# WGLab/NanoRepeat

Hardware: NVIDIA B200
Metric: GCUPS (higher is better)
Workload: dtype u16x2 (2*score + mark + 64 per half, two reads per word); s32 (score*65536 - span) for reads > 384 bases

## Files before the change

include/nanorepeat_b200.h:

```cpp
#ifndef NANOREPEAT_B200_H
#define NANOREPEAT_B200_H

#include <stdint.h>

#ifdef __cplusplus
extern "C" {
#endif

#define NR_OK                0
#define NR_ERR_CUDA         -1
#define NR_ERR_ARG          -2
#define NR_ERR_BAD_BASE     -3
#define NR_ERR_TOO_LARGE    -4
#define NR_ERR_NOMEM        -5
#define NR_ERR_UNKNOWN_TYPE -6

typedef struct nr_scoring_t {
    int32_t match;
    int32_t mismatch;
    int32_t gap_open1;
    int32_t gap_ext1;
    int32_t gap_open2;
    int32_t gap_ext2;
    int32_t ambiguous;
// ... 10 lines not shown
} nr_rung_t;

typedef struct nr_stats_t {
    int64_t algorithmic_cells;
    int64_t executed_cells;
    int64_t n_tasks;
    int32_t kernel_launches;
    int32_t n_skipped;
    int64_t h2d_bytes;
    int64_t d2h_bytes;
} nr_stats_t;

typedef struct nr_launch_info_t {
    int64_t paired_cells;
    int64_t rest_cells;
    int32_t n_pairs;
    int32_t n_rest;
    int32_t n_redo;
    int32_t reserved;
    float paired_ms, rest_ms, redo_ms;
    float reserved2;
    int64_t paired_useful_cells;
    int64_t rest_useful_cells;
} nr_launch_info_t;

int nr_get_preset(const char* data_type, nr_scoring_t* out);

int nr_init(int device);
int nr_shutdown(void);
const char* nr_last_error(void);
int nr_device_info(int32_t* device, int32_t* sm_count, int32_t* clock_khz);

int nr_limits(int32_t* max_score, int32_t* max_tlen);

int nr_set_ladder_mode(int mode);

int nr_score_tasks(const nr_scoring_t* sc, int32_t n_tasks,
                   const char* const* queries, const int32_t* qlen,
                   const char* const* targets, const int32_t* tlen,
                   nr_aln_t* out);

int nr_round2_region(const nr_scoring_t* sc,
                     const char* left, int32_t n_left, const char* motif, int32_t motif_len, int32_t T,
                     int32_t n_reads, const char* const* cores, const int32_t* core_len,
                     nr_aln_t* out);

// ... 97 lines not shown
```

nanorepeat_b200/csrc/nr_api.cu:

```cuda
#include "../../include/nanorepeat_b200.h"
#include "nr_launch.h"

#include <algorithm>
#if defined(__x86_64__)
#include <tmmintrin.h>
#endif
#include <atomic>
#include <chrono>
#include <cstdarg>
#include <cstdio>
#include <cstdlib>
#include <cstring>
#include <functional>
#include <mutex>
#include <new>
#include <string>
#include <thread>
#include <memory>
#include <unordered_map>
#include <vector>

namespace {

thread_local std::string g_err;
thread_local int g_code = 0;
thread_local nr_stats_t g_last_stats = {};
// ... 242 lines not shown
    std::vector<nr::Task> tasks;
    std::vector<nr::LadderTask> ltasks;
    std::vector<nr::LadderRegion> lregs;
    bool ladder = false;
    bool flag = false;
    bool pair = false;
    bool r2flags = false;
    std::vector<nr::pr::Pair2> pairs2;
    std::vector<nr::pr::Pair3> pairs3;
    int n_pairs2_single = 0, n_pairs3_single = 0;
    bool long_redone = false;
    int n_long_pairs = 0;
    void* d_pairs = nullptr;
    uint2* d_prung = nullptr;
    size_t prung_bytes = 0;
    int32_t* d_redo = nullptr;
    size_t redo_bytes = 0;
    cudaEvent_t ev_t[6] = {};
    bool timed[3] = {};
    int* h_redo_count = nullptr;
    int* h_spin = nullptr;
    long long paired_cells = 0, rest_cells = 0;
    long long paired_useful = 0, rest_useful = 0;
    size_t n_out = 0;
    std::vector<int32_t> order;
    std::vector<nr::CoopInfo> coop;
    std::vector<int32_t> coop_idx;
    nr::CoopInfo* d_coop = nullptr;
    int32_t* d_coop_idx = nullptr;
    std::vector<int32_t> lt_src;
    uint32_t* d_state = nullptr;
    size_t state_bytes = 0;
    int* d_flags = nullptr;
    size_t flags_bytes = 0;
    Launch launch = {};
    Pool pool;
    std::vector<RegionInfo> regions;
    int n_reads = 0;
    int n_skipped = 0;
    int n_ambiguous_reads = 0;
    std::vector<int32_t> read_region;
    std::vector<int32_t> kmin, kmax;
    std::vector<int64_t> rung_off;
    void* d_blob = nullptr;
    size_t blob_bytes = 0;
    void* h_blob = nullptr;
    nr::Task* d_tasks = nullptr;
    nr::LadderTask* d_ltasks = nullptr;
    nr::LadderRegion* d_lregs = nullptr;
    int32_t* d_order = nullptr;
    uint32_t* d_pool = nullptr;
    int* d_counters = nullptr;
    int4* d_out = nullptr;
    size_t out_bytes = 0;
// ... 52 lines not shown
    return k;
}

size_t align_up(size_t x, size_t a) { return (x + a - 1) / a * a; }

struct PhaseTrace {
    const bool on = getenv("NR_TRACE") != nullptr;
    std::chrono::steady_clock::time_point t0 = std::chrono::steady_clock::now();
    void mark(const char* what) {
        if (!on) return;
        const auto t1 = std::chrono::steady_clock::now();
        fprintf(stderr, "[nr trace] %-28s %8.1f us   (ends at %10.1f us, thread %04x)\n", what,
                std::chrono::duration<double, std::micro>(t1 - t0).count(), std::fmod(std::chrono::duration<double, std::micro>(t1.time_since_epoch()).count(), 1e8),
                (unsigned)(std::hash<std::thread::id>()(std::this_thread::get_id()) & 0xffff));
        t0 = t1;
    }
};

bool is_map_ont(const nr_scoring_t& c) {
    return c.match == 2 && c.mismatch == 4 && c.gap_open1 == 4 && c.gap_ext1 == 2 && c.gap_open2 == 24 && c.gap_ext2 == 1 &&
           c.ambiguous == 1;
}

template <class Key, class Emit>
void make_pairs(std::vector<int>& ids, Key key, Emit emit) {
    std::vector<uint64_t> w(ids.size());
    for (size_t i = 0; i < ids.size(); ++i) w[i] = ((uint64_t)(uint32_t)key(ids[i]) << 32) | (uint32_t)~(uint32_t)ids[i];
    std::sort(w.begin(), w.end(), std::greater<uint64_t>());
    for (size_t i = 0; i < w.size(); ++i) ids[i] = (int)~(uint32_t)w[i];
    for (size_t i = 0; i < ids.size(); i += 2) emit(ids[i], i + 1 < ids.size() ? ids[i + 1] : -1);
}

int plan_batch(nr_batch* b) {
    const bool ladder = b->ladder;
    const int n = ladder ? (int)b->ltasks.size() : (int)b->tasks.size();
    if (b->kind != KIND_ROUND3) b->n_out = b->tasks.size();
    b->stats = {};
    b->stats.n_tasks = (int64_t)b->n_out;
    std::vector<long long> cost(n, 0);
    std::vector<int> task_R(n, nr::kMinR), task_ns(n, 1), task_sweep(n, 0), task_rungs(n, 0);
    std::vector<char> paired(n, 0);
    const int max_r = ladder ? nr::kMaxRLadder : nr::kMaxRExact;
    const bool fixed = is_map_ont(b->sc);
    PhaseTrace trace;
    for (int i = 0; i < n; ++i) {
        int q_len, t_len, t_sweep;
// ... 11 lines not shown
        } else {
            const nr::Task& t = b->tasks[i];
            q_len = t.q_len;
            t_len = t_sweep = t.t_len;
            if (t_len > 0) b->stats.algorithmic_cells += (long long)q_len * t_len;
        }
        if (q_len <= 0 || t_len <= 0) {
            paired[i] = 2;
            if (t_len < 0) ++b->n_skipped;
            continue;
        }
        long long m = (long long)b->sc.match * std::min(q_len, t_len);
        if (m > kMaxScore || t_len > kMaxTlen) {
            paired[i] = 2;
            ++b->n_skipped;
            continue;
        }
        nr::stripe_shape(q_len, max_r, task_R[i], task_ns[i]);
        task_sweep[i] = t_sweep;
        cost[i] = (long long)task_ns[i] * 32 * task_R[i] * t_len;
    }
    trace.mark("task shapes");
    std::vector<long long> pair_cost;
    Launch& L = b->launch;
    L = {};
    long long state_off = 0;
    long long rung_off = 0;
    if (b->pair && fixed && !ladder && b->kind == KIND_ROUND2) {
        for (const RegionInfo& g : b->regions) {
            std::vector<int> ids;
            for (int r = g.first_read; r < g.first_read + g.n_reads; ++r) {
                const nr::Task& t = b->tasks[r];
                if (!paired[r] && t.q_len >= 1 && t.q_len <= 32 * nr::pr::kMaxRPair2 && t.t_len >= 1) ids.push_back(r);
            }
            make_pairs(ids, [&](int i) { return b->tasks[i].q_len; }, [&](int x, int y) {
                const int R = nr::pr::pair_rows(b->tasks[x].q_len);
                nr::pr::Pair2 p = {x, y, g.n_left, -1};
                if (g.n_left >= 2 && state_off + nr::pr::state_words(R) < 0x7fffffffLL) {
                    p.state_off = (int32_t)state_off;
                    state_off += nr::pr::state_words(R);
                }
                b->pairs2.push_back(p);
                paired[x] = 1;
                if (y >= 0) paired[y] = 1;
                L.pair_R = std::max(L.pair_R, R);
                pair_cost.push_back((long long)32 * R * b->tasks[x].t_len);
                b->paired_useful += (long long)(b->tasks[x].q_len + (y >= 0 ? b->tasks[y].q_len : 0)) * b->tasks[x].t_len;
            });
        }
    } else if (b->pair && fixed && ladder && b->flag) {
        if (b->qsrc && !b->qsrc->pairs2.empty() && (int)b->lt_src.size() == n) {
            const nr_batch* src = b->qsrc;
            std::vector<int> src2lt(src->tasks.size(), -1);
            for (int i = 0; i < n; ++i)
                if (b->lt_src[i] >= 0) src2lt[b->lt_src[i]] = i;
            for (int pi = 0; pi < src->n_pairs2_single; ++pi) {
                const nr::pr::Pair2& p2 = src->pairs2[pi];
                int la = src2lt[p2.a], lb = p2.b >= 0 ? src2lt[p2.b] : -1;
                if (la >= 0 && paired[la]) la = -1;
                if (lb >= 0 && paired[lb]) lb = -1;
                if (la < 0 && lb < 0) continue;
                const nr::LadderRegion& g = b->lregs[b->ltasks[la >= 0 ? la : lb].region];
                if (g.n_left <= 0 || g.n_right <= 0) continue;
                const int q = std::max(src->tasks[p2.a].q_len, p2.b >= 0 ? src->tasks[p2.b].q_len : 0);
                const int R = nr::pr::pair_rows(q);
                int kmin = INT32_MAX, kmax = -1;
                for (int t : {la, lb})
                    if (t >= 0) { kmin = std::min(kmin, b->ltasks[t].kmin); kmax = std::max(kmax, b->ltasks[t].kmax); }
                nr::pr::Pair3 p = {la, lb, (int32_t)rung_off, -1, R, {0, 0, 0}};
                if (p2.state_off >= 0 && src->d_state && g.n_left >= 2 && g.n_left == p2.mark_col) p.state_off = p2.state_off;
// ... 21 lines not shown
                if (y >= 0) { kmin = std::min(kmin, b->ltasks[y].kmin); kmax = std::max(kmax, b->ltasks[y].kmax); }
                nr::pr::Pair3 p = {x, y, (int32_t)rung_off, -1, 0, {0, 0, 0}};
                rung_off += kmax - kmin + 1;
                b->pairs3.push_back(p);
                paired[x] = 1;
                if (y >= 0) paired[y] = 1;
                const int R = nr::pr::pair_rows(tx.q_len);
                L.pair_R = std::max(L.pair_R, R);
                pair_cost.push_back((long long)32 * R * (g.n_right + g.n_left + (long long)g.m * kmax));
                b->paired_useful += (long long)(tx.q_len + (y >= 0 ? b->ltasks[y].q_len : 0)) * (g.n_right + g.n_left + (long long)g.m * kmax);
            });
            i0 = i1;
        }
        if (rung_off > 0x7fffffffLL) return fail(NR_ERR_TOO_LARGE, "more than 2^31 rungs in one batch");
        L.redo_R = L.pair_R;
    }
    trace.mark("pairing");
    b->state_bytes = sizeof(uint32_t) * 32 * (size_t)state_off;
    L.n_pairs = (int)pair_cost.size();
    if (L.n_pairs) {
        std::vector<int> po(L.n_pairs);
        {
            std::vector<uint64_t> w(L.n_pairs);
            for (int i = 0; i < L.n_pairs; ++i) w[i] = ((uint64_t)pair_cost[i] << 24) | (uint32_t)(0xffffff - i);
            std::sort(w.begin(), w.end(), std::greater<uint64_t>());
            for (int i = 0; i < L.n_pairs; ++i) po[i] = 0xffffff - (int)(w[i] & 0xffffff);
        }
        if (!b->pairs2.empty()) { std::vector<nr::pr::Pair2> t(L.n_pairs); for (int i = 0; i < L.n_pairs; ++i) t[i] = b->pairs2[po[i]]; b->pairs2.swap(t); }
        else { std::vector<nr::pr::Pair3> t(L.n_pairs); for (int i = 0; i < L.n_pairs; ++i) t[i] = b->pairs3[po[i]]; b->pairs3.swap(t); }
        for (long long c : pair_cost) b->paired_cells += 2 * c;
        b->stats.executed_cells += b->paired_cells;
        L.pair_blocks = std::max(1, std::min(g_ctx.sm_count, L.n_pairs));
    }
    trace.mark("pair order");
    b->n_pairs2_single = (int)b->pairs2.size();
    struct LongPair { int a, b, n_left; long long cost; };
    std::vector<LongPair> long_pairs;
    long long long_pair_rows = 0;
    b->n_pairs3_single = (int)b->pairs3.size();
    if (b->pair && fixed && ladder && b->flag && !getenv("NR_NO_LONG_PAIRS")) {
        for (int i0 = 0; i0 < n;) {
            int i1 = i0;
            while (i1 < n && b->ltasks[i1].region == b->ltasks[i0].region) ++i1;
            const nr::LadderRegion& g = b->lregs[b->ltasks[i0].region];
            std::vector<int> ids;
            if (g.n_left > 0 && g.n_right > 0)
                for (int i = i0; i < i1; ++i)
// ... 216 lines not shown
    const size_t order_bytes = sizeof(int32_t) * n_rest;
    const size_t pair_bytes = b->pairs2.empty() ? sizeof(nr::pr::Pair3) * b->pairs3.size() : sizeof(nr::pr::Pair2) * b->pairs2.size();
    const size_t pool_bytes = sizeof(uint32_t) * (b->pool.words.size() + 4);
    const size_t coop_bytes = sizeof(nr::CoopInfo) * b->coop.size();
    const size_t cidx_bytes = b->coop.empty() ? 0 : sizeof(int32_t) * b->coop_idx.size();
    const size_t off_reg = align_up(task_bytes, 256);
    const size_t off_order = off_reg + align_up(reg_bytes, 256);
    const size_t off_pair = off_order + align_up(order_bytes, 256);
    const size_t off_coop = off_pair + align_up(pair_bytes, 256);
    const size_t off_cidx = off_coop + align_up(coop_bytes, 256);
    const size_t off_pool = off_cidx + align_up(cidx_bytes, 256);
    const size_t off_cnt = off_pool + align_up(pool_bytes, 256);
    b->blob_bytes = off_cnt + 256;
    b->out_bytes = sizeof(int4) * std::max<size_t>(b->n_out, 1);
    b->scratch_bytes = sizeof(int4) * scratch_total;
    int rc;
    if ((rc = cached_alloc(&b->d_blob, b->blob_bytes, BUF_DEV))) return rc;
    if ((rc = cached_alloc(&b->h_blob, b->blob_bytes, BUF_PIN))) return rc;
    if ((rc = cached_alloc((void**)&b->d_out, b->out_bytes, BUF_DEV))) return rc;
    if ((rc = cached_alloc((void**)&b->h_out, b->out_bytes, BUF_PIN))) return rc;
    if (scratch_total && (rc = cached_alloc((void**)&b->d_scratch, b->scratch_bytes, BUF_SCRATCH))) return rc;
    if (b->flags_bytes && (rc = cached_alloc((void**)&b->d_flags, b->flags_bytes, BUF_DEV))) return rc;
    if (b->state_bytes && (rc = cached_alloc((void**)&b->d_state, b->state_bytes, BUF_DEV))) return rc;
    if (b->flag) {
        b->sel_bytes = sizeof(int4) * std::max<size_t>((size_t)b->n_reads, 1);
        if ((rc = cached_alloc((void**)&b->d_sel, b->sel_bytes, BUF_DEV))) return rc;
        if ((rc = cached_alloc((void**)&b->h_sel, b->sel_bytes, BUF_PIN))) return rc;
    }
    if (!b->pairs3.empty()) {
        b->redo_bytes = sizeof(int32_t) * (size_t)n * 2;
        if ((rc = cached_alloc((void**)&b->d_prung, b->prung_bytes, BUF_DEV))) return rc;
        if ((rc = cached_alloc((void**)&b->d_redo, b->redo_bytes, BUF_DEV))) return rc;
        if ((rc = cached_alloc((void**)&b->h_redo_count, 64, BUF_PIN))) return rc;
        b->h_redo_count[0] = b->h_redo_count[1] = 0;
    }
    trace.mark("buffers (cached alloc)");
    char* h = static_cast<char*>(b->h_blob);
    char* d = static_cast<char*>(b->d_blob);
    if (task_bytes) memcpy(h, ladder ? (const void*)b->ltasks.data() : (const void*)b->tasks.data(), task_bytes);
    if (reg_bytes) memcpy(h + off_reg, b->lregs.data(), reg_bytes);
    if (order_bytes) memcpy(h + off_order, b->order.data(), order_bytes);
    if (coop_bytes) memcpy(h + off_coop, b->coop.data(), coop_bytes);
    if (cidx_bytes) memcpy(h + off_cidx, b->coop_idx.data(), cidx_bytes);
    if (pair_bytes) memcpy(h + off_pair, b->pairs2.empty() ? (const void*)b->pairs3.data() : (const void*)b->pairs2.data(), pair_bytes);
    if (!b->pool.words.empty()) memcpy(h + off_pool, b->pool.words.data(), pool_bytes - 16);
    memset(h + off_pool + pool_bytes - 16, 0, 16);
// ... 97 lines not shown
        if (b->qsrc->run_stream != st) CUDA_TRY(cudaStreamWaitEvent(st, b->qsrc->ev_done, 0));
    }
    CUDA_TRY(cudaMemsetAsync(b->d_counters, 0, 32 * sizeof(int), st));
    if (b->flags_bytes) CUDA_TRY(cudaMemsetAsync(b->d_flags, 0, b->flags_bytes, st));
    int launches = 0;
    int rc;
    const bool timing = g_timing.load() != 0;
    if (timing)
        for (cudaEvent_t& e : b->ev_t)
            if (!e) CUDA_TRY(cudaEventCreate(&e));
    b->timed[0] = b->timed[1] = b->timed[2] = false;
    auto mark = [&](int i, cudaStream_t s) { return timing ? cudaEventRecord(b->ev_t[i], s) : cudaSuccess; };
    if (L.n_pairs || b->n_long_pairs) {
        const bool ladder_batch = L.ladder;
        nr::RestArgs ra;
        if ((rc = rest_args(b, b->d_order, L.count, st, &ra))) return rc;
        int wpb = kWarpsPerBlock;
        if (const char* e = getenv("NR_WPB")) wpb = std::max(4, std::min(kWarpsPerBlock, atoi(e)));
        const int blocks = std::max(1, std::min(g_ctx.sm_count, L.count + L.n_pairs));
        nr::pr::Deal deal = nr::pr::make_deal(L.count, L.n_pairs, wpb, blocks);
        if (getenv("NR_PLAIN_DEAL")) deal.nb_long = -1;
        CUDA_TRY(mark(2, st));
        if (!ladder_batch) {
            const int stride = exact_smem_int4(std::max(L.pair_R, L.R));
            const size_t smem = (size_t)wpb * stride * sizeof(int4);
            if (smem > nrl::kMaxDynShared) return fail(NR_ERR_ARG, "launch needs %zu bytes of shared memory", smem);
            CUDA_TRY(nrl::launch_pair_round2(blocks, wpb * 32, smem, st, static_cast<const nr::pr::Pair2*>(b->d_pairs), deal, b->d_tasks,
                                             ra, b->d_pool, k, b->d_counters, stride, b->d_out, b->d_state));
        } else {
            const int stride = pair_ladder_smem_int4(L.pair_R, L.R);
            const size_t smem = (size_t)wpb * stride * sizeof(int4);
            if (smem > nrl::kMaxDynShared) return fail(NR_ERR_ARG, "launch needs %zu bytes of shared memory", smem);
            CUDA_TRY(nrl::launch_pair_ladder(blocks, wpb * 32, smem, st, static_cast<const nr::pr::Pair3*>(b->d_pairs), deal, b->d_ltasks,
                                             ra, b->qsrc ? b->qsrc->d_pool : b->d_pool, b->d_pool, b->d_lregs, k, b->d_counters, stride,
                                             b->d_prung, b->d_out, b->d_sel, b->d_counters + 2, b->d_redo,
                                             b->qsrc ? b->qsrc->d_state : nullptr));
        }
        CUDA_TRY(cudaGetLastError());
        CUDA_TRY(mark(3, st));
        b->timed[1] = timing;
        ++launches;
        if (!b->pairs3.empty()) {
            CUDA_TRY(mark(4, st));
            if ((rc = launch_rest(b, st, k, b->d_redo, 0, std::max(1, std::min(g_ctx.sm_count, 2 * L.n_pairs)), L.redo_R,
                                  b->d_counters + 2, b->d_counters + 3))) return rc;
            CUDA_TRY(mark(5, st));
            b->timed[2] = timing;
            CUDA_TRY(cudaMemcpyAsync(b->h_redo_count, b->d_counters + 2, sizeof(int), cudaMemcpyDeviceToHost, st));
            CUDA_TRY(cudaMemcpyAsync(b->h_redo_count + 1, b->d_counters + 4, sizeof(int), cudaMemcpyDeviceToHost, st));
            ++launches;
        }
// ... 356 lines not shown
    g_ladder_mode.store(mode);
    return NR_OK;
}

int nr_limits(int32_t* max_score, int32_t* max_tlen) {
    if (max_score) *max_score = kMaxScore;
    if (max_tlen) *max_tlen = kMaxTlen;
    return NR_OK;
}

void nr_batch_destroy(nr_batch_t* b) {
    if (!b) return;
    if (--b->refs > 0) return;
    if (b->committed && b->ev_uploaded) cudaEventSynchronize(b->ev_uploaded);
    if (b->ran && b->ev_done) cudaEventSynchronize(b->ev_done);
    else if (b->ran && b->run_stream) cudaStreamSynchronize(b->run_stream);
    cached_free(b->d_blob, b->blob_bytes, BUF_DEV);
    cached_free(b->h_blob, b->blob_bytes, BUF_PIN);
    cached_free(b->d_out, b->out_bytes, BUF_DEV);
    cached_free(b->h_out, b->out_bytes, BUF_PIN);
    cached_free(b->d_scratch, b->scratch_bytes, BUF_SCRATCH);
    cached_free(b->d_flags, b->flags_bytes, BUF_DEV);
    cached_free(b->d_state, b->state_bytes, BUF_DEV);
    cached_free(b->d_sel, b->sel_bytes, BUF_DEV);
    cached_free(b->h_sel, b->sel_bytes, BUF_PIN);
    cached_free(b->d_prung, b->prung_bytes, BUF_DEV);
    cached_free(b->d_redo, b->redo_bytes, BUF_DEV);
    cached_free(b->h_redo_count, 64, BUF_PIN);
    cached_free(b->h_spin, 64, BUF_PIN);
    nr_batch* src = b->qsrc;
    free_events(b);
    delete b;
    if (src) nr_batch_destroy(src);
}

nr_batch_t* nr_batch_begin_round3_from(nr_batch_t* round2) {
    if (!round2 || round2->kind != KIND_ROUND2 || !round2->committed) {
        fail(NR_ERR_ARG, "nr_batch_begin_round3_from: needs a committed round-2 batch");
        return nullptr;
    }
    nr_batch* b = new_batch(&round2->sc, KIND_ROUND3);
    if (!b) return nullptr;
    if (!b->ladder) {
        fail(NR_ERR_ARG, "nr_batch_begin_round3_from: needs a ladder mode (nr_set_ladder_mode 1 or 2)");
        free_events(b);
        delete b;
// ... 223 lines not shown
                rg.score = a.x;
                rg.starts_in_left = in_left;
                rg.ends_in_right = in_right;
                rg.pad[0] = rg.pad[1] = 0;
            }
            if (top > 0 && a.x == top && in_left) { sum += k; ++cnt; }
        }
        sum_k[r] = sum;
        n_k[r] = cnt;
        top_score[r] = top;
    }
    return NR_OK;
}

int nr_set_timing(int on) {
    g_timing.store(on ? 1 : 0);
    return NR_OK;
}

int nr_batch_launch_info(nr_batch_t* b, nr_launch_info_t* out) {
    if (!b || !out) return fail(NR_ERR_ARG, "nr_batch_launch_info: NULL argument");
    if (!b->committed) return fail(NR_ERR_ARG, "nr_batch_launch_info: batch was not committed");
    *out = {};
    out->paired_cells = b->paired_cells;
    out->rest_cells = b->rest_cells;
    out->paired_useful_cells = b->paired_useful;
    out->rest_useful_cells = b->rest_useful;
    out->n_pairs = b->launch.n_pairs;
    out->n_rest = b->launch.count;
    if (b->ran) {
        CUDA_TRY(cudaEventSynchronize(b->ev_done));
        if (b->h_redo_count) out->n_redo = *b->h_redo_count;
        if (b->timed[0]) CUDA_TRY(cudaEventElapsedTime(&out->rest_ms, b->ev_t[0], b->ev_t[1]));
        if (b->timed[1]) CUDA_TRY(cudaEventElapsedTime(&out->paired_ms, b->ev_t[2], b->ev_t[3]));
        if (b->timed[2]) CUDA_TRY(cudaEventElapsedTime(&out->redo_ms, b->ev_t[4], b->ev_t[5]));
    }
    return NR_OK;
}

int nr_batch_stats(const nr_batch_t* b, nr_stats_t* out) {
    if (!b || !out) return fail(NR_ERR_ARG, "nr_batch_stats: NULL argument");
    *out = b->stats;
    return NR_OK;
}

int nr_last_stats(nr_stats_t* out) {
    if (!out) return fail(NR_ERR_ARG, "nr_last_stats: NULL argument");
    *out = g_last_stats;
    return NR_OK;
}

int nr_score_tasks(const nr_scoring_t* sc, int32_t n_tasks, const char* const* queries, const int32_t* qlen,
                   const char* const* targets, const int32_t* tlen, nr_aln_t* out) {
    if (n_tasks > 0 && !out) return fail(NR_ERR_ARG, "nr_score_tasks: out is NULL");
// ... 295 lines not shown
```

nanorepeat_b200/csrc/nr_launch.h:

```cpp
#pragma once
#include "nr_kernels.cuh"
#include "nr_pair_kernels.cuh"

namespace nrl {

constexpr size_t kMaxDynShared = (size_t)nr::kWarpsPerBlock * 14 * 1024;

cudaError_t launch_exact(bool fixed, int blocks, int threads, size_t smem, cudaStream_t st, const nr::Task* tasks,
                         const nr::RestArgs& ra, const uint32_t* pool, const nr::ScoreW& k, int* counter, int stride, int4* out);
cudaError_t launch_ladder(bool flag, int blocks, int threads, size_t smem, cudaStream_t st, const nr::LadderTask* tasks,
                          const nr::RestArgs& ra, const int* n_order_dev, const uint32_t* qpool, const uint32_t* pool,
                          const nr::LadderRegion* regs, const nr::ScoreW& k, int* counter, int stride, int4* out, int4* sel);
cudaError_t launch_pair_round2(int blocks, int threads, size_t smem, cudaStream_t st, const nr::pr::Pair2* pairs,
                               const nr::pr::Deal& deal, const nr::Task* tasks, const nr::RestArgs& ra, const uint32_t* pool,
                               const nr::ScoreW& k, int* counter, int stride, int4* out, uint32_t* state);
cudaError_t launch_pair_ladder(int blocks, int threads, size_t smem, cudaStream_t st, const nr::pr::Pair3* pairs,
                               const nr::pr::Deal& deal, const nr::LadderTask* tasks, const nr::RestArgs& ra,
                               const uint32_t* qpool, const uint32_t* pool, const nr::LadderRegion* regs, const nr::ScoreW& k,
                               int* counter, int stride, uint2* prung, int4* out, int4* sel, int* redo_count, int32_t* redo,
                               const uint32_t* qstate);

template <class F>
inline cudaError_t prepare(F fn, bool& done) {
    if (done) return cudaSuccess;
    cudaError_t e = cudaFuncSetAttribute(fn, cudaFuncAttributeMaxDynamicSharedMemorySize, (int)kMaxDynShared);
    if (e == cudaSuccess) e = cudaFuncSetAttribute(fn, cudaFuncAttributePreferredSharedMemoryCarveout, cudaSharedmemCarveoutMaxShared);
    if (e == cudaSuccess) done = true;
    return e;
}

}
```

nanorepeat_b200/csrc/nr_launch_pair2.cu:

```cuda
#define NR_DEFINE_PAIR_ROUND2_KERNEL
#include "nr_launch.h"
#include <mutex>
namespace nrl {
cudaError_t launch_pair_round2(int blocks, int threads, size_t smem, cudaStream_t st, const nr::pr::Pair2* pairs,
                               const nr::pr::Deal& deal, const nr::Task* tasks, const nr::RestArgs& ra, const uint32_t* pool,
                               const nr::ScoreW& k, int* counter, int stride, int4* out, uint32_t* state) {
    static std::mutex mu;
    static bool done = false;
    {
        std::lock_guard<std::mutex> lk(mu);
        cudaError_t e = prepare(nr::pr::pair_round2_kernel, done);
        if (e != cudaSuccess) return e;
    }
    nr::pr::pair_round2_kernel<<<blocks, threads, smem, st>>>(pairs, deal, tasks, ra, pool, k, counter, stride, out, state);
    return cudaGetLastError();
}
}
```

nanorepeat_b200/csrc/nr_pair_kernels.cuh:

```cuda
#pragma once
#include "nr_kernels.cuh"

namespace nr {
namespace pr {

typedef unsigned u32;
constexpr int kBias = 64;
__host__ __device__ constexpr u32 pk2(int hi, int lo) { return ((u32)(hi & 0xffff) << 16) | (u32)(lo & 0xffff); }
__host__ __device__ constexpr u32 pk(int v) { return pk2(v, v); }
__host__ __device__ constexpr u32 sub2(int v) { return 0u - (((u32)v << 16) | (u32)v); }

constexpr int kMatch = 4, kMismatch = 8, kAmbiguous = 2, kOpen1 = 12, kExt1 = 4, kOpen2 = 50, kExt2 = 2, kRefund1 = 8, kRefund2 = 48;
constexpr u32 kFloorFwd = pk(kBias + 1);
constexpr u32 kFloorBwd = pk(kBias);
constexpr u32 kOnes = 0x00010001u;

__device__ __forceinline__ u32 pmadd(u32 a, u32 mul, u32 b) {
    u32 d;
    asm("mad.lo.u32 %0, %1, %2, %3;" : "=r"(d) : "r"(a), "r"(mul), "r"(b));
    return d;
}

template <u32 FLOOR>
__device__ __forceinline__ void cell(u32 hd, u32 s, u32 one, u32& h, u32& e1, u32& e2, u32& f1, u32& f2) {
    const u32 d = __viaddmax_u16x2(hd, s, FLOOR);
    const u32 t = __vimax3_u16x2(d, e1, e2);
    h = __vimax3_u16x2(t, f1, f2);
    e1 = __viaddmax_u16x2(h, pk(-kOpen1), pmadd(e1, one, sub2(kExt1)));
    e2 = __viaddmax_u16x2(h, pk(-kOpen2), pmadd(e2, one, sub2(kExt2)));
    f1 = __viaddmax_u16x2(h, pk(-kOpen1), pmadd(f1, one, sub2(kExt1)));
    f2 = __viaddmax_u16x2(h, pk(-kOpen2), pmadd(f2, one, sub2(kExt2)));
}

struct Pair2 {
    int32_t a, b;
    int32_t mark_col;
    int32_t state_off;
};

struct Pair3 {
    int32_t a, b;
    int32_t rung_off;
    int32_t state_off;
    int32_t R;
    int32_t pad[3];
};

__host__ __device__ constexpr int state_words(int R) { return 3 * R + 1; }

template <int R>
__device__ __forceinline__ void build_profile(uint4* prof, const uint32_t* __restrict__ qa, int q_a,
                                              const uint32_t* __restrict__ qb, int q_b, int row0, int lane, bool reverse) {
    constexpr int CH = StripeCfg<R>::CH;
    u32* p = reinterpret_cast<u32*>(prof);
    const uint32_t amb_a = q_a > 0 ? read_ambiguity_plane(qa, q_a) : 0u, amb_b = q_b > 0 ? read_ambiguity_plane(qb, q_b) : 0u;
#pragma unroll
    for (int r = 0; r < 4 * CH; ++r) {
        const int i = row0 + r;
        int ca = 4, cb = 4;
        if (r < R && i < q_a) {
            const int qi = reverse ? q_a - 1 - i : i;
// ... 25 lines not shown
    int* spin;
    int4 bcur;
    ulonglong2 bnxt;
    const ulonglong2* tok_in;
    ulonglong2* tok_out;
    const u32* bstage;
    int b_stride, brow0;
    const int* bdone;
    int bdone_need;
    bool late_pending;
    u32* bsm_w;
    const uint4* prof;
    const uint32_t* twords;
    int t_len, lane;
    int mark_col;
    int q_a, q_b;
    const u32* bsm;
    uint2* rung_out;
    int jnext, m, kcnt, zone_start;
    int col0;
    const u32* resume;
    u32* save;
    int save_col;
    u32 H[R], E1[R], E2[R];
    u32 hup_prev, h_out, f1_out, f2_out;
    u32 best;
    u32 bestc, raw_hi, raw_lo;
    int st_hi, st_lo;
    u32 nz, bz;
    uint32_t twl, w0, w1;
    int wi, wmax, wsh;
    const char* prof_lane;
    u32 tokP, tokJ;

    __device__ __forceinline__ uint32_t tword(int i) const { return __ldg(&twords[min(max(i, 0), wmax)]); }

    __device__ __forceinline__ void init() {
        if (MODE == kPF && resume) {
#pragma unroll
            for (int r = 0; r < R; ++r) {
                H[r] = __ldcg(&resume[r * 32 + lane]);
                E1[r] = __ldcg(&resume[(R + r) * 32 + lane]);
                E2[r] = __ldcg(&resume[(2 * R + r) * 32 + lane]);
            }
            hup_prev = lane ? __ldcg(&resume[(R - 1) * 32 + lane - 1]) : FLOOR;
            best = __ldcg(&resume[3 * R * 32 + lane]);
// ... 224 lines not shown
            if (MULTI && bot && lane == 31) store_bnd(&bnd_out[jj], (int)h_out, (int)f1_out, (int)f2_out, tag_out);
        }
    }

    __device__ __forceinline__ void slow_until(int& st, int end, u32 one, unsigned four) {
#pragma unroll 1
        for (; st < end; ++st) {
            if (MULTI && MODE == kPF && late_pending && st >= zone_start) late_load();
            if ((st & 15) == 0) refill();
            step<false, true>(st, one, four);
        }
    }

#ifndef NR_PAIR3_UNROLL
#define NR_PAIR3_UNROLL 2
#endif
#ifndef NR_PAIR2_UNROLL
#define NR_PAIR2_UNROLL 4
#endif
#ifndef NR_PAIR2_MULTI_UNROLL
#define NR_PAIR2_MULTI_UNROLL 4
#endif
    static constexpr int kUnroll = MODE == kP2 ? (MULTI ? NR_PAIR2_MULTI_UNROLL : NR_PAIR2_UNROLL) : (MULTI ? 1 : NR_PAIR3_UNROLL);
    template <bool TRACK, bool SPECIAL = false>
    __device__ __forceinline__ void fast_until(int& st, int end, u32 one, unsigned four) {
        for (; st + 16 <= end; st += 16) {
            refill();
#pragma unroll 1
            for (int b = 0; b < 16; b += kUnroll) {
#pragma unroll
                for (int u = 0; u < kUnroll; ++u) step<true, TRACK, SPECIAL>(st + b + u, one, four);
            }
        }
    }

    __device__ __forceinline__ void run(u32 one, unsigned four, int zone_start_) {
        init();
        zone_start = zone_start_;
        const int n = t_len - col0;
        const int nsteps = n + 31;
        const int inside_end = ((n - 1) >> 4) << 4;
        const int mc = mark_col - col0;
        int st = 0;
        slow_until(st, min(32, nsteps), one, four);
        if (MODE == kPB) {
            fast_until<true>(st, inside_end, one, four);
        } else if (MODE == kP2) {
            if (mc >= 0) {
                const int zs = max(mc - 2, 0);
                const int before = st;
                fast_until<false>(st, min(inside_end, (zs >> 4) << 4), one, four);
                if (st != before) {
                    const u32 nb = __vmaxu2(bestc, best | kOnes);
                    const u32 x = nb ^ bestc;
                    bestc = nb;
                    if (x > 0xffffu) { st_hi = lane; raw_hi = 0; }
                    if (x & 0xffffu) { st_lo = lane; raw_lo = 0; }
                }
                slow_until(st, min(nsteps, ((mc + 32 + 15) >> 4) << 4), one, four);
            }
            fast_until<true>(st, inside_end, one, four);
        } else {
            const int first = min(zone_start, mc >= 0 ? mc : zone_start);
            fast_until<true>(st, min(inside_end, (first >> 4) << 4), one, four);
            if (MULTI && late_pending && st + 16 <= inside_end) late_load();
            fast_until<true, true>(st, inside_end, one, four);
        }
        slow_until(st, nsteps, one, four);
    }
};

constexpr int kMaxRPair3 = 16;
constexpr int kMaxRPair2 = kMaxRPair3;
constexpr int kPairEntry = 1 << 30;

__host__ __device__ __forceinline__ int pair_rows(int q_len) {
    int R = (q_len + 31) / 32;
    return R < kMinR ? kMinR : R;
}

struct Deal {
    int n_rest, n_pairs;
    int static_rest;
    int nb_long;
// ... 23 lines not shown
    }
    if (first) {
        first = false;
        const int wpb = blockDim.x >> 5, warp = threadIdx.x >> 5, blk = (int)blockIdx.x;
        if (blk < dl.nb_long) {
            const int e = blk * wpb + warp;
            if (e < dl.static_rest) return e;
        } else {
            const int p = warp * ((int)gridDim.x - dl.nb_long) + (blk - dl.nb_long);
            if (p < dl.static_pairs) return dl.n_rest + p;
        }
    }
    int d = 0;
    if ((threadIdx.x & 31) == 0) d = atomicAdd(counter, 1);
    d = __shfl_sync(kFull, d, 0);
    const int rest_left = dl.n_rest - dl.static_rest;
    if (d < rest_left) return dl.static_rest + d;
    const int p = dl.static_pairs + d - rest_left;
    return p < dl.n_pairs ? dl.n_rest + p : -1;
}

template <int R>
__device__ __forceinline__ void pair2_task(const Pair2& pt, const Task* __restrict__ tasks, const uint32_t* __restrict__ pool,
                                           uint4* prof, int lane, u32 one, unsigned four, int4* out, u32* state) {
    const Task ta = tasks[pt.a];
    Task tb = ta;
    int q_b = 0;
    if (pt.b >= 0) { tb = tasks[pt.b]; q_b = tb.q_len; }
    __syncwarp();
    build_profile<R>(prof, pool + ta.q_word, ta.q_len, pool + tb.q_word, q_b, lane * R, lane, false);
    __syncwarp();
    Sweep<R, kP2> sw;
    sw.prof = prof; sw.twords = pool + ta.t_word; sw.t_len = ta.t_len; sw.lane = lane;
    sw.mark_col = pt.mark_col;
    sw.col0 = 0; sw.resume = nullptr;
    sw.save_col = pt.mark_col - 2;
    sw.save = (state && pt.state_off >= 0 && sw.save_col >= 0) ? state + (size_t)pt.state_off * 32 : nullptr;
    sw.run(one, four, 0);
#pragma unroll
    for (int half = 0; half < 2; ++half) {
        const u32 cls = half ? (sw.bestc & 0xffffu) : (sw.bestc >> 16);
        const u32 raw = half ? (sw.raw_lo & 0xffffu) : (sw.raw_hi >> 16);
        const int st = half ? sw.st_lo : sw.st_hi;
        const int score = (int)(cls - (kBias + 1)) >> 1;
        const int col = st - lane;
        unsigned key = 0;
        if (score > 0) key = ((unsigned)score << 17) | ((0xffffu - (unsigned)col) << 1) | (raw & 1u);
        key = __reduce_max_sync(kFull, key);
        const int tid = half ? pt.b : pt.a;
        if (lane == 0 && tid >= 0) {
            int4 rec = make_int4(0, 0, 0, 0);
            if (key) {
                const int c = 0xffff - (int)((key >> 1) & 0xffffu);
                const bool inside = c <= pt.mark_col || !(key & 1u);
                rec = make_int4((int)(key >> 17), inside ? 0 : pt.mark_col + 1, c + 1, 0);
            }
            out[tid] = rec;
        }
    }
}

// ... 47 lines not shown
                if (key) {
                    const int c = 0xffff - (int)((key >> 1) & 0xffffu);
                    const bool inside = c <= pt.mark_col || !(key & 1u);
                    rec = make_int4((int)(key >> 17), inside ? 0 : pt.mark_col + 1, c + 1, 0);
                }
                out[tid] = rec;
            }
        }
    }
}

template <int R>
__device__ __forceinline__ void pair2_stripe_dispatch(int r, const Pair2& pt, int s, const Task* __restrict__ tasks,
                                                      const uint32_t* __restrict__ pool, const RestArgs& ra, uint4* prof, int lane,
                                                      u32 one, unsigned four, int4* out) {
    if constexpr (is_coop_height(R))
        if (r == R) { pair2_stripe<R>(pt, s, tasks, pool, ra, prof, lane, one, four, out); return; }
    if constexpr (R < kMaxRLadder) pair2_stripe_dispatch<R + 1>(r, pt, s, tasks, pool, ra, prof, lane, one, four, out);
}

template <int R>
__device__ __forceinline__ void pair2_dispatch(int r, const Pair2& pt, const Task* __restrict__ tasks,
                                               const uint32_t* __restrict__ pool, uint4* prof, int lane, u32 one,
                                               unsigned four, int4* out, u32* state) {
    if (r == R) { pair2_task<R>(pt, tasks, pool, prof, lane, one, four, out, state); return; }
    if constexpr (R < kMaxRPair2) pair2_dispatch<R + 1>(r, pt, tasks, pool, prof, lane, one, four, out, state);
}

#ifdef NR_DEFINE_PAIR_ROUND2_KERNEL
__global__ void __launch_bounds__(32 * kWarpsPerBlock, 1)
pair_round2_kernel(const Pair2* __restrict__ pairs, Deal dl, const Task* __restrict__ tasks, RestArgs ra,
                   const uint32_t* __restrict__ pool, ScoreW scw, int* counter, int smem_stride, int4* out, u32* state) {
    extern __shared__ uint4 psmem[];
    const ScoreView<true> sc(scw);
    const int lane = threadIdx.x & 31, warp = threadIdx.x >> 5;
    uint4* prof = psmem + warp * smem_stride;
    bool first = true;
    for (;;) {
        const int i = next_item(dl, first, counter);
        if (i < 0) break;
        if (i < ra.n_order) {
            const int e = ra.order[i];
            if (e & kPairEntry) {
                const Pair2 mp = pairs[(e & ~kPairEntry) >> kCodeBits];
                pair2_stripe_dispatch<kMinR>(ra.coop[mp.state_off].rows, mp, (e & ((1 << kCodeBits) - 1)) - 1, tasks, pool, ra, prof, lane,
                                             (u32)sc.one, sc.four, out);
            } else {
                exact_entry(e, tasks, pool, sc, ra, reinterpret_cast<int4*>(prof), lane, out);
            }
            continue;
        }
        const Pair2 pt = pairs[i - ra.n_order];
        int q = tasks[pt.a].q_len;
        if (pt.b >= 0) q = max(q, tasks[pt.b].q_len);
        pair2_dispatch<kMinR>(pair_rows(q), pt, tasks, pool, prof, lane, (u32)sc.one, sc.four, out, state);
    }
}
#endif

__device__ __forceinline__ void rung_of(u32 P, u32 J, u32 rc, int& score, bool& in_right, bool& unmarked) {
    const u32 np = max(J, rc);
    const int s_p = (int)(P - kBias) >> 1;
    const int s_np = (int)(np - 2 * kBias) >> 1;
    in_right = s_np > s_p;
    score = max(s_p, s_np);
    unmarked = np & 1u;
}

__device__ __forceinline__ void pair3_select(const Pair3& pt, const LadderTask& ta, const LadderTask& tb, int kmin, u32 rcand,
                                             const uint2* rungs, int lane, int min_score, int4* sel, int* redo_count, int32_t* redo,
                                             int redo_shift) {
#pragma unroll
    for (int half = 0; half < 2; ++half) {
        const int tid = half ? pt.b : pt.a;
        if (tid < 0) continue;
        const LadderTask& tk = half ? tb : ta;
        const u32 rc = half ? (rcand & 0xffffu) : (rcand >> 16);
        int top = 0;
// ... 227 lines not shown
```

nanorepeat_b200/engine.py:

```python
import ctypes
import itertools
import os

import numpy as np

_HERE = os.path.dirname(os.path.abspath(__file__))
LIB_PATH = os.path.join(_HERE, "libnanorepeat_b200.so")

NR_OK = 0
ERROR_NAMES = {-1: "NR_ERR_CUDA", -2: "NR_ERR_ARG", -3: "NR_ERR_BAD_BASE", -4: "NR_ERR_TOO_LARGE",
               -5: "NR_ERR_NOMEM", -6: "NR_ERR_UNKNOWN_TYPE"}


class Scoring(ctypes.Structure):
    _fields_ = [(n, ctypes.c_int32) for n in
                ("match", "mismatch", "gap_open1", "gap_ext1", "gap_open2", "gap_ext2", "ambiguous", "min_dp_score")]


class Stats(ctypes.Structure):
    _fields_ = [("algorithmic_cells", ctypes.c_int64), ("executed_cells", ctypes.c_int64),
                ("n_tasks", ctypes.c_int64), ("kernel_launches", ctypes.c_int32), ("n_skipped", ctypes.c_int32),
                ("h2d_bytes", ctypes.c_int64), ("d2h_bytes", ctypes.c_int64)]

    def as_dict(self):
        return {n: int(getattr(self, n)) for n, _ in self._fields_ if n != "reserved"}


class LaunchInfo(ctypes.Structure):
    _fields_ = [("paired_cells", ctypes.c_int64), ("rest_cells", ctypes.c_int64), ("n_pairs", ctypes.c_int32),
                ("n_rest", ctypes.c_int32), ("n_redo", ctypes.c_int32), ("reserved", ctypes.c_int32),
                ("paired_ms", ctypes.c_float), ("rest_ms", ctypes.c_float), ("redo_ms", ctypes.c_float),
                ("reserved2", ctypes.c_float), ("paired_useful_cells", ctypes.c_int64), ("rest_useful_cells", ctypes.c_int64)]

    def as_dict(self):
        return {n: getattr(self, n) for n, _ in self._fields_ if not n.startswith("reserved")}


class RegionIn(ctypes.Structure):
    _fields_ = [("left", ctypes.c_char_p), ("n_left", ctypes.c_int32), ("right", ctypes.c_char_p), ("n_right", ctypes.c_int32),
                ("motif", ctypes.c_char_p), ("motif_len", ctypes.c_int32), ("n_reads", ctypes.c_int32),
                ("reads", ctypes.c_void_p), ("reads_len", ctypes.c_int64),
                ("dist_between_anchors", ctypes.POINTER(ctypes.c_int32)),
                ("has_round1_max_dist", ctypes.c_int32), ("round1_max_dist", ctypes.c_int64)]


ALN_DTYPE = np.dtype([("score", "<i4"), ("tstart", "<i4"), ("tend", "<i4")])
RUNG_DTYPE = np.dtype([("score", "<i4"), ("starts_in_left", "u1"), ("ends_in_right", "u1"), ("pad", "u1", (2,))])


class GmmParams(ctypes.Structure):
    _fields_ = [("max_components", ctypes.c_int32), ("n_init", ctypes.c_int32), ("max_iter", ctypes.c_int32),
                ("reserved", ctypes.c_int32), ("error_rate", ctypes.c_double), ("max_mutual_overlap", ctypes.c_double),
                ("tol", ctypes.c_double), ("reg_covar", ctypes.c_double), ("seed", ctypes.c_uint64)]

    def __init__(self, error_rate=0.03, max_mutual_overlap=0.15, max_components=22, seed=0, n_init=10, max_iter=100, tol=1e-3,
# ... 525 lines not shown
```

Baseline: 65740.

## Exit round-2 paired DP early once the column state repeats with the motif period

Adds a periodic check in the round-2 paired fast loop. After a check column, the warp compares its boundary and stripe state against a snapshot taken one motif period earlier, kept in global scratch and in shared memory. If the new state is dominated by the snapshot, it stops computing the remaining columns. Pairs are now dealt by a predicted post-exit cost rather than the full target length. This adds snapshot loads, stores and a warp vote at each check, plus extra shared memory. Its correctness rests on the periodic-dominance argument, and it is on by default via NR_ROUND2_EXIT.

```diff
diff --git a/include/nanorepeat_b200.h b/include/nanorepeat_b200.h
--- a/include/nanorepeat_b200.h
+++ b/include/nanorepeat_b200.h
@@ -56,6 +56,8 @@
     float reserved2;
     int64_t paired_useful_cells;
     int64_t rest_useful_cells;
+    int64_t planned_paired_cells;
+    int64_t planned_paired_useful_cells;
 } nr_launch_info_t;
 
 int nr_get_preset(const char* data_type, nr_scoring_t* out);
diff --git a/nanorepeat_b200/csrc/nr_api.cu b/nanorepeat_b200/csrc/nr_api.cu
--- a/nanorepeat_b200/csrc/nr_api.cu
+++ b/nanorepeat_b200/csrc/nr_api.cu
@@ -2,6 +2,7 @@
 #include "nr_launch.h"
 
 #include <algorithm>
+#include <numeric>
 #if defined(__x86_64__)
 #include <tmmintrin.h>
 #endif
@@ -290,6 +291,7 @@
     int* h_spin = nullptr;
     long long paired_cells = 0, rest_cells = 0;
     long long paired_useful = 0, rest_useful = 0;
+    bool round2_exit = false;
     size_t n_out = 0;
     std::vector<int32_t> order;
     std::vector<nr::CoopInfo> coop;
@@ -298,6 +300,7 @@
     int32_t* d_coop_idx = nullptr;
     std::vector<int32_t> lt_src;
     uint32_t* d_state = nullptr;
+    uint32_t* d_kept = nullptr;
     size_t state_bytes = 0;
     int* d_flags = nullptr;
     size_t flags_bytes = 0;
@@ -396,6 +399,13 @@
            c.ambiguous == 1;
 }
 
+bool round2_exit_enabled() {
+    const char* e = getenv("NR_ROUND2_EXIT");
+    return !(e && atoi(e) == 0);
+}
+int round2_check_col(int n_left, int q_len) { return std::max(n_left + 1, n_left + q_len - 192); }
+int round2_predicted_exit(int n_left, int q_len) { return n_left + std::max(q_len - 64, 32); }
+
 template <class Key, class Emit>
 void make_pairs(std::vector<int>& ids, Key key, Emit emit) {
     std::vector<uint64_t> w(ids.size());
@@ -453,11 +463,13 @@
     }
     trace.mark("task shapes");
     std::vector<long long> pair_cost;
+    std::vector<long long> deal_cost;
     Launch& L = b->launch;
     L = {};
     long long state_off = 0;
     long long rung_off = 0;
     if (b->pair && fixed && !ladder && b->kind == KIND_ROUND2) {
+        const bool exits = round2_exit_enabled();
         for (const RegionInfo& g : b->regions) {
             std::vector<int> ids;
             for (int r = g.first_read; r < g.first_read + g.n_reads; ++r) {
@@ -466,7 +478,15 @@
             }
             make_pairs(ids, [&](int i) { return b->tasks[i].q_len; }, [&](int x, int y) {
                 const int R = nr::pr::pair_rows(b->tasks[x].q_len);
-                nr::pr::Pair2 p = {x, y, g.n_left, -1};
+                nr::pr::Pair2 p = {x, y, g.n_left, -1, -1, 0, {0, 0}};
+                const int t_len = b->tasks[x].t_len;
+                int cols = t_len;
+                if (exits) {
+                    p.check_col = round2_check_col(g.n_left, b->tasks[x].q_len);
+                    p.period = 16 / std::gcd(16, g.motif_len) * g.motif_len;
+                    cols = std::min(t_len, round2_predicted_exit(g.n_left, b->tasks[x].q_len));
+                    b->round2_exit = true;
+                }
                 if (g.n_left >= 2 && state_off + nr::pr::state_words(R) < 0x7fffffffLL) {
                     p.state_off = (int32_t)state_off;
                     state_off += nr::pr::state_words(R);
@@ -475,8 +495,9 @@
                 paired[x] = 1;
                 if (y >= 0) paired[y] = 1;
                 L.pair_R = std::max(L.pair_R, R);
-                pair_cost.push_back((long long)32 * R * b->tasks[x].t_len);
-                b->paired_useful += (long long)(b->tasks[x].q_len + (y >= 0 ? b->tasks[y].q_len : 0)) * b->tasks[x].t_len;
+                pair_cost.push_back((long long)32 * R * t_len);
+                deal_cost.push_back((long long)32 * R * cols);
+                b->paired_useful += (long long)(b->tasks[x].q_len + (y >= 0 ? b->tasks[y].q_len : 0)) * t_len;
             });
         }
     } else if (b->pair && fixed && ladder && b->flag) {
@@ -544,7 +565,8 @@
         std::vector<int> po(L.n_pairs);
         {
             std::vector<uint64_t> w(L.n_pairs);
-            for (int i = 0; i < L.n_pairs; ++i) w[i] = ((uint64_t)pair_cost[i] << 24) | (uint32_t)(0xffffff - i);
+            const std::vector<long long>& dc = deal_cost.empty() ? pair_cost : deal_cost;
+            for (int i = 0; i < L.n_pairs; ++i) w[i] = ((uint64_t)dc[i] << 24) | (uint32_t)(0xffffff - i);
             std::sort(w.begin(), w.end(), std::greater<uint64_t>());
             for (int i = 0; i < L.n_pairs; ++i) po[i] = 0xffffff - (int)(w[i] & 0xffffff);
         }
@@ -807,6 +829,8 @@
     if (scratch_total && (rc = cached_alloc((void**)&b->d_scratch, b->scratch_bytes, BUF_SCRATCH))) return rc;
     if (b->flags_bytes && (rc = cached_alloc((void**)&b->d_flags, b->flags_bytes, BUF_DEV))) return rc;
     if (b->state_bytes && (rc = cached_alloc((void**)&b->d_state, b->state_bytes, BUF_DEV))) return rc;
+    if (b->round2_exit &&
+        (rc = cached_alloc((void**)&b->d_kept, sizeof(uint32_t) * 128 * kWarpsPerBlock * (size_t)g_ctx.sm_count, BUF_DEV))) return rc;
     if (b->flag) {
         b->sel_bytes = sizeof(int4) * std::max<size_t>((size_t)b->n_reads, 1);
         if ((rc = cached_alloc((void**)&b->d_sel, b->sel_bytes, BUF_DEV))) return rc;
@@ -950,11 +974,12 @@
         if (getenv("NR_PLAIN_DEAL")) deal.nb_long = -1;
         CUDA_TRY(mark(2, st));
         if (!ladder_batch) {
-            const int stride = exact_smem_int4(std::max(L.pair_R, L.R));
+            const int stride = std::max(exact_smem_int4(std::max(L.pair_R, L.R)),
+                                        b->round2_exit ? exact_smem_int4(L.pair_R) + 3 * L.pair_R * 8 : 0);
             const size_t smem = (size_t)wpb * stride * sizeof(int4);
             if (smem > nrl::kMaxDynShared) return fail(NR_ERR_ARG, "launch needs %zu bytes of shared memory", smem);
             CUDA_TRY(nrl::launch_pair_round2(blocks, wpb * 32, smem, st, static_cast<const nr::pr::Pair2*>(b->d_pairs), deal, b->d_tasks,
-                                             ra, b->d_pool, k, b->d_counters, stride, b->d_out, b->d_state));
+                                             ra, b->d_pool, k, b->d_counters, stride, b->d_out, b->d_state, b->d_kept));
         } else {
             const int stride = pair_ladder_smem_int4(L.pair_R, L.R);
             const size_t smem = (size_t)wpb * stride * sizeof(int4);
@@ -1357,6 +1382,7 @@
     cached_free(b->d_scratch, b->scratch_bytes, BUF_SCRATCH);
     cached_free(b->d_flags, b->flags_bytes, BUF_DEV);
     cached_free(b->d_state, b->state_bytes, BUF_DEV);
+    if (b->d_kept) cached_free(b->d_kept, sizeof(uint32_t) * 128 * kWarpsPerBlock * (size_t)g_ctx.sm_count, BUF_DEV);
     cached_free(b->d_sel, b->sel_bytes, BUF_DEV);
     cached_free(b->h_sel, b->sel_bytes, BUF_PIN);
     cached_free(b->d_prung, b->prung_bytes, BUF_DEV);
@@ -1626,14 +1652,20 @@
     if (!b || !out) return fail(NR_ERR_ARG, "nr_batch_launch_info: NULL argument");
     if (!b->committed) return fail(NR_ERR_ARG, "nr_batch_launch_info: batch was not committed");
     *out = {};
-    out->paired_cells = b->paired_cells;
+    out->paired_cells = out->planned_paired_cells = b->paired_cells;
     out->rest_cells = b->rest_cells;
-    out->paired_useful_cells = b->paired_useful;
+    out->paired_useful_cells = out->planned_paired_useful_cells = b->paired_useful;
     out->rest_useful_cells = b->rest_useful;
     out->n_pairs = b->launch.n_pairs;
     out->n_rest = b->launch.count;
     if (b->ran) {
         CUDA_TRY(cudaEventSynchronize(b->ev_done));
+        if (b->round2_exit) {
+            unsigned long long skipped[2];
+            CUDA_TRY(cudaMemcpy(skipped, b->d_counters + nr::pr::kExitSlot, sizeof(skipped), cudaMemcpyDeviceToHost));
+            out->paired_cells -= 2 * (int64_t)skipped[0];
+            out->paired_useful_cells -= (int64_t)(skipped[1] / 32);
+        }
         if (b->h_redo_count) out->n_redo = *b->h_redo_count;
         if (b->timed[0]) CUDA_TRY(cudaEventElapsedTime(&out->rest_ms, b->ev_t[0], b->ev_t[1]));
         if (b->timed[1]) CUDA_TRY(cudaEventElapsedTime(&out->paired_ms, b->ev_t[2], b->ev_t[3]));
diff --git a/nanorepeat_b200/csrc/nr_launch.h b/nanorepeat_b200/csrc/nr_launch.h
--- a/nanorepeat_b200/csrc/nr_launch.h
+++ b/nanorepeat_b200/csrc/nr_launch.h
@@ -13,7 +13,8 @@
                           const nr::LadderRegion* regs, const nr::ScoreW& k, int* counter, int stride, int4* out, int4* sel);
 cudaError_t launch_pair_round2(int blocks, int threads, size_t smem, cudaStream_t st, const nr::pr::Pair2* pairs,
                                const nr::pr::Deal& deal, const nr::Task* tasks, const nr::RestArgs& ra, const uint32_t* pool,
-                               const nr::ScoreW& k, int* counter, int stride, int4* out, uint32_t* state);
+                               const nr::ScoreW& k, int* counter, int stride, int4* out, uint32_t* state,
+                               uint32_t* kept);
 cudaError_t launch_pair_ladder(int blocks, int threads, size_t smem, cudaStream_t st, const nr::pr::Pair3* pairs,
                                const nr::pr::Deal& deal, const nr::LadderTask* tasks, const nr::RestArgs& ra,
                                const uint32_t* qpool, const uint32_t* pool, const nr::LadderRegion* regs, const nr::ScoreW& k,
diff --git a/nanorepeat_b200/csrc/nr_launch_pair2.cu b/nanorepeat_b200/csrc/nr_launch_pair2.cu
--- a/nanorepeat_b200/csrc/nr_launch_pair2.cu
+++ b/nanorepeat_b200/csrc/nr_launch_pair2.cu
@@ -4,7 +4,8 @@
 namespace nrl {
 cudaError_t launch_pair_round2(int blocks, int threads, size_t smem, cudaStream_t st, const nr::pr::Pair2* pairs,
                                const nr::pr::Deal& deal, const nr::Task* tasks, const nr::RestArgs& ra, const uint32_t* pool,
-                               const nr::ScoreW& k, int* counter, int stride, int4* out, uint32_t* state) {
+                               const nr::ScoreW& k, int* counter, int stride, int4* out, uint32_t* state,
+                               uint32_t* kept) {
     static std::mutex mu;
     static bool done = false;
     {
@@ -12,7 +13,7 @@
         cudaError_t e = prepare(nr::pr::pair_round2_kernel, done);
         if (e != cudaSuccess) return e;
     }
-    nr::pr::pair_round2_kernel<<<blocks, threads, smem, st>>>(pairs, deal, tasks, ra, pool, k, counter, stride, out, state);
+    nr::pr::pair_round2_kernel<<<blocks, threads, smem, st>>>(pairs, deal, tasks, ra, pool, k, counter, stride, out, state, kept);
     return cudaGetLastError();
 }
 }
diff --git a/nanorepeat_b200/csrc/nr_pair_kernels.cuh b/nanorepeat_b200/csrc/nr_pair_kernels.cuh
--- a/nanorepeat_b200/csrc/nr_pair_kernels.cuh
+++ b/nanorepeat_b200/csrc/nr_pair_kernels.cuh
@@ -36,7 +36,12 @@
     int32_t a, b;
     int32_t mark_col;
     int32_t state_off;
+    int32_t check_col;
+    int32_t period;
+    int32_t pad[2];
 };
+
+constexpr int kExitSlot = 24;
 
 struct Pair3 {
     int32_t a, b;
@@ -108,6 +113,11 @@
     const u32* resume;
     u32* save;
     int save_col;
+    bool exits;
+    int check_col, period;
+    int next_check;
+    int exit_st;
+    u32* kept_io;
     u32 H[R], E1[R], E2[R];
     u32 hup_prev, h_out, f1_out, f2_out;
     u32 best;
@@ -378,9 +388,13 @@
 #define NR_PAIR2_MULTI_UNROLL 4
 #endif
     static constexpr int kUnroll = MODE == kP2 ? (MULTI ? NR_PAIR2_MULTI_UNROLL : NR_PAIR2_UNROLL) : (MULTI ? 1 : NR_PAIR3_UNROLL);
-    template <bool TRACK, bool SPECIAL = false>
+    template <bool TRACK, bool SPECIAL = false, bool EXIT = false>
     __device__ __forceinline__ void fast_until(int& st, int end, u32 one, unsigned four) {
         for (; st + 16 <= end; st += 16) {
+            if (EXIT && st == next_check) {
+                if (dominated_then_keep()) { exit_st = st; return; }
+                next_check += (int)__ldcg(kept_io + 96 + lane);
+            }
             refill();
 #pragma unroll 1
             for (int b = 0; b < 16; b += kUnroll) {
@@ -390,9 +404,26 @@
         }
     }
 
+    __device__ __forceinline__ bool dominated_then_keep() {
+        u32* g = kept_io + lane;
+        const u32 khp = __ldcg(g), kf1 = __ldcg(g + 32), kf2 = __ldcg(g + 64);
+        u32 acc = (__vmaxu2(hup_prev, khp) ^ khp) | (__vmaxu2(f1_out, kf1) ^ kf1) | (__vmaxu2(f2_out, kf2) ^ kf2);
+        __stcg(g, hup_prev); __stcg(g + 32, f1_out); __stcg(g + 64, f2_out);
+        u32* snap = reinterpret_cast<u32*>(const_cast<uint4*>(prof) + StripeCfg<R>::PROF_INT4);
+#pragma unroll
+        for (int r = 0; r < R; ++r) {
+            u32* k = snap + r * 32 + lane;
+            const u32 kh = k[0], ke1 = k[R * 32], ke2 = k[2 * R * 32];
+            acc |= (__vmaxu2(H[r], kh) ^ kh) | (__vmaxu2(E1[r], ke1) ^ ke1) | (__vmaxu2(E2[r], ke2) ^ ke2);
+            k[0] = H[r]; k[R * 32] = E1[r]; k[2 * R * 32] = E2[r];
+        }
+        return __all_sync(kFull, acc == 0);
+    }
+
     __device__ __forceinline__ void run(u32 one, unsigned four, int zone_start_) {
         init();
         zone_start = zone_start_;
+        exit_st = -1;
         const int n = t_len - col0;
         const int nsteps = n + 31;
         const int inside_end = ((n - 1) >> 4) << 4;
@@ -415,7 +446,19 @@
                 }
                 slow_until(st, min(nsteps, ((mc + 32 + 15) >> 4) << 4), one, four);
             }
-            fast_until<true>(st, inside_end, one, four);
+            if (MULTI) {
+                fast_until<true>(st, inside_end, one, four);
+            } else {
+                next_check = -1;
+                if (exits && mc >= 0) {
+                    const int c0 = max(st, ((check_col - col0 + 32 + 15) >> 4) << 4);
+                    if (c0 + period < inside_end) next_check = c0;
+                    __stcg(kept_io + lane, 0u); __stcg(kept_io + 32 + lane, 0u); __stcg(kept_io + 64 + lane, 0u);
+                    __stcg(kept_io + 96 + lane, (u32)period);
+                }
+                fast_until<true, false, true>(st, inside_end, one, four);
+                if (exit_st >= 0) return;
+            }
         } else {
             const int first = min(zone_start, mc >= 0 ? mc : zone_start);
             fast_until<true>(st, min(inside_end, (first >> 4) << 4), one, four);
@@ -485,7 +528,8 @@
 
 template <int R>
 __device__ __forceinline__ void pair2_task(const Pair2& pt, const Task* __restrict__ tasks, const uint32_t* __restrict__ pool,
-                                           uint4* prof, int lane, u32 one, unsigned four, int4* out, u32* state) {
+                                           uint4* prof, int lane, u32 one, unsigned four, int4* out, u32* state,
+                                           unsigned long long* skipped, u32* kept) {
     const Task ta = tasks[pt.a];
     Task tb = ta;
     int q_b = 0;
@@ -499,7 +543,15 @@
     sw.col0 = 0; sw.resume = nullptr;
     sw.save_col = pt.mark_col - 2;
     sw.save = (state && pt.state_off >= 0 && sw.save_col >= 0) ? state + (size_t)pt.state_off * 32 : nullptr;
+    sw.exits = pt.check_col >= 0;
+    sw.check_col = pt.check_col; sw.period = pt.period;
+    sw.kept_io = kept + (size_t)((blockIdx.x * (blockDim.x >> 5) + (threadIdx.x >> 5)) * 128);
     sw.run(one, four, 0);
+    if (sw.exit_st >= 0 && lane == 0) {
+        const unsigned long long cols32 = 32ull * (unsigned)ta.t_len - (32ull * (unsigned)sw.exit_st - 496ull);
+        atomicAdd(&skipped[0], (unsigned long long)R * cols32);
+        atomicAdd(&skipped[1], (unsigned long long)(ta.q_len + q_b) * cols32);
+    }
 #pragma unroll
     for (int half = 0; half < 2; ++half) {
         const u32 cls = half ? (sw.bestc & 0xffffu) : (sw.bestc >> 16);
@@ -593,15 +645,16 @@
 template <int R>
 __device__ __forceinline__ void pair2_dispatch(int r, const Pair2& pt, const Task* __restrict__ tasks,
                                                const uint32_t* __restrict__ pool, uint4* prof, int lane, u32 one,
-                                               unsigned four, int4* out, u32* state) {
-    if (r == R) { pair2_task<R>(pt, tasks, pool, prof, lane, one, four, out, state); return; }
-    if constexpr (R < kMaxRPair2) pair2_dispatch<R + 1>(r, pt, tasks, pool, prof, lane, one, four, out, state);
+                                               unsigned four, int4* out, u32* state, unsigned long long* skipped, u32* kept) {
+    if (r == R) { pair2_task<R>(pt, tasks, pool, prof, lane, one, four, out, state, skipped, kept); return; }
+    if constexpr (R < kMaxRPair2) pair2_dispatch<R + 1>(r, pt, tasks, pool, prof, lane, one, four, out, state, skipped, kept);
 }
 
 #ifdef NR_DEFINE_PAIR_ROUND2_KERNEL
 __global__ void __launch_bounds__(32 * kWarpsPerBlock, 1)
 pair_round2_kernel(const Pair2* __restrict__ pairs, Deal dl, const Task* __restrict__ tasks, RestArgs ra,
-                   const uint32_t* __restrict__ pool, ScoreW scw, int* counter, int smem_stride, int4* out, u32* state) {
+                   const uint32_t* __restrict__ pool, ScoreW scw, int* counter, int smem_stride, int4* out, u32* state,
+                   u32* kept) {
     extern __shared__ uint4 psmem[];
     const ScoreView<true> sc(scw);
     const int lane = threadIdx.x & 31, warp = threadIdx.x >> 5;
@@ -624,7 +677,8 @@
         const Pair2 pt = pairs[i - ra.n_order];
         int q = tasks[pt.a].q_len;
         if (pt.b >= 0) q = max(q, tasks[pt.b].q_len);
-        pair2_dispatch<kMinR>(pair_rows(q), pt, tasks, pool, prof, lane, (u32)sc.one, sc.four, out, state);
+        pair2_dispatch<kMinR>(pair_rows(q), pt, tasks, pool, prof, lane, (u32)sc.one, sc.four, out, state,
+                              reinterpret_cast<unsigned long long*>(counter + kExitSlot), kept);
     }
 }
 #endif
diff --git a/nanorepeat_b200/engine.py b/nanorepeat_b200/engine.py
--- a/nanorepeat_b200/engine.py
+++ b/nanorepeat_b200/engine.py
@@ -30,7 +30,8 @@
     _fields_ = [("paired_cells", ctypes.c_int64), ("rest_cells", ctypes.c_int64), ("n_pairs", ctypes.c_int32),
                 ("n_rest", ctypes.c_int32), ("n_redo", ctypes.c_int32), ("reserved", ctypes.c_int32),
                 ("paired_ms", ctypes.c_float), ("rest_ms", ctypes.c_float), ("redo_ms", ctypes.c_float),
-                ("reserved2", ctypes.c_float), ("paired_useful_cells", ctypes.c_int64), ("rest_useful_cells", ctypes.c_int64)]
+                ("reserved2", ctypes.c_float), ("paired_useful_cells", ctypes.c_int64), ("rest_useful_cells", ctypes.c_int64),
+                ("planned_paired_cells", ctypes.c_int64), ("planned_paired_useful_cells", ctypes.c_int64)]
 
     def as_dict(self):
         return {n: getattr(self, n) for n, _ in self._fields_ if not n.startswith("reserved")}
```

Result: faster. 69690 (median of 6 runs) (+6.0%).
